# InternRobotics/InternNav

Measured on AMD Instinct MI355X. Metric: policy steps/sec/node, higher is better.
Workload: dtype bf16

## Files before the change

internnav_amd/csrc/gemm_skinny.hip:

```cpp
#include "gemm_skinny_core.h"

namespace {

struct SkBf16 {
    static constexpr bool ROW_SCALE = false;
    using Q = void;
    using S = void;

    template <int MF, int NT16, int NW, int DEPTH>
    static __device__ __forceinline__ void main_fused(const GemmArgs& p, const void*, const void*, int n0, int w, int nmine, int r16, int g,
                                                      f32x4 (&acc)[NT16][MF]) {
        const bf16* __restrict__ A = reinterpret_cast<const bf16*>(p.A);
        const bf16* __restrict__ W = reinterpret_cast<const bf16*>(p.W);
        const bf16x8 zero8 = {0, 0, 0, 0, 0, 0, 0, 0};
        const bf16* wrow[NT16];
        bool wok[NT16];
#pragma unroll
        for (int t = 0; t < NT16; ++t) {
            const int wn = n0 + t * 16 + r16;
            wok[t] = wn < p.N;
            wrow[t] = W + (size_t)(wok[t] ? wn : 0) * p.ldw;
        }
        const bf16* arow[MF];
        bool aok[MF];
#pragma unroll
        for (int i = 0; i < MF; ++i) {
            const int m = i * 16 + r16;
            aok[i] = m < p.M;
            arow[i] = A + (size_t)(aok[i] ? m : 0) * p.lda;
        }
        bf16x8 wf[DEPTH][NT16][4], af[DEPTH][MF][4];
        auto load = [&](int j, int slot) {
            const int k0 = (w + j * NW) * SK_BK + g * 8;
#pragma unroll
            for (int s = 0; s < 4; ++s) {
                const int k = k0 + s * 32;
                const bool kok = j < nmine && k < p.K;
#pragma unroll
                for (int t = 0; t < NT16; ++t) wf[slot][t][s] = (kok && wok[t]) ? *reinterpret_cast<const bf16x8*>(wrow[t] + k) : zero8;
#pragma unroll
                for (int i = 0; i < MF; ++i) af[slot][i][s] = (kok && aok[i]) ? *reinterpret_cast<const bf16x8*>(arow[i] + k) : zero8;
            }
        };
#pragma unroll
        for (int d = 0; d < DEPTH; ++d) load(d, d);
        for (int j0 = 0; j0 < nmine; j0 += DEPTH) {
#pragma unroll
            for (int d = 0; d < DEPTH; ++d) {
#pragma unroll
                for (int t = 0; t < NT16; ++t)
#pragma unroll
                    for (int i = 0; i < MF; ++i)
#pragma unroll
                        for (int s = 0; s < 4; ++s) acc[t][i] = __builtin_amdgcn_mfma_f32_16x16x32_bf16(wf[d][t][s], af[d][i][s], acc[t][i], 0, 0, 0);
                load(j0 + d + DEPTH, d);
            }
        }
    }

    template <int NT16, int NW, int DEPTH, class Norm>
    static __device__ __forceinline__ void main_prenorm(const GemmArgs& p, const void*, const void*, const bf16* img, int lds_ld, int n0, int w,
                                                        int nmine, int r16, int g, f32x4 (&acc)[NT16][1], Norm norm) {
        const bf16* __restrict__ W = reinterpret_cast<const bf16*>(p.W);
        const bf16x8 zero8 = {0, 0, 0, 0, 0, 0, 0, 0};
        const bf16* wrow[NT16];
        bool wok[NT16];
#pragma unroll
        for (int t = 0; t < NT16; ++t) {
            const int wn = n0 + t * 16 + r16;
            wok[t] = wn < p.N;
            wrow[t] = W + (size_t)(wok[t] ? wn : 0) * p.ldw;
        }
        bf16x8 wf[DEPTH][NT16][4];
        auto load_w = [&](int j, int slot) {
            const int k0 = (w + j * NW) * SK_BK + g * 8;
#pragma unroll
            for (int s = 0; s < 4; ++s) {
                const int k = k0 + s * 32;
                const bool kok = j < nmine && k < p.K;
#pragma unroll
                for (int t = 0; t < NT16; ++t) wf[slot][t][s] = (kok && wok[t]) ? *reinterpret_cast<const bf16x8*>(wrow[t] + k) : zero8;
            }
        };
#pragma unroll
        for (int d = 0; d < DEPTH; ++d) load_w(d, d);
        norm();
        const bf16* arow = img + (size_t)(r16 < p.M ? r16 : p.M - 1) * lds_ld + g * 8;
        for (int j0 = 0; j0 < nmine; j0 += DEPTH) {
#pragma unroll
            for (int d = 0; d < DEPTH; ++d) {
                const int kb = (w + (j0 + d) * NW) * SK_BK;
#pragma unroll
                for (int s = 0; s < 4; ++s) {
                    const int k = kb + s * 32;
                    const bf16x8 af = (j0 + d < nmine && k + g * 8 < p.K) ? *reinterpret_cast<const bf16x8*>(arow + k) : zero8;
#pragma unroll
                    for (int t = 0; t < NT16; ++t) acc[t][0] = __builtin_amdgcn_mfma_f32_16x16x32_bf16(wf[d][t][s], af, acc[t][0], 0, 0, 0);
                }
                load_w(j0 + d + DEPTH, d);
            }
        }
    }
};

}

int ina_launch_gemm_skinny_fused(const GemmArgs& p, hipStream_t stream) {
    InaProfScope prof(INA_PROF_GEMM_SKINNY, 2.0 * p.M * p.N * p.K, sk_prof_bytes(p, 2.0 * p.N * p.K), stream);
    return sk_launch_fused<SkBf16>(p, nullptr, nullptr, stream);
}

int ina_launch_gemm_skinny_prenorm(const GemmArgs& p, hipStream_t stream) {
// ... 4 lines not shown
```

internnav_amd/csrc/gemm_skinny_core.h:

```cpp
#pragma once
#include "common.h"
#include "kernels.h"

namespace {

constexpr int SK_BK = 128;

inline int sk_group_waves(int tiles, int ksteps) {
    int nw = tiles >= 4096 ? 1 : tiles >= 2048 ? 2 : tiles >= 1024 ? 4 : 8;
    while (nw > 1 && nw > ksteps) nw >>= 1;
    return nw;
}
inline int sk_group_waves_prenorm(int tiles, int ksteps) {
    const int nw = sk_group_waves(tiles, ksteps);
    return nw < 4 ? 4 : nw;
}

template <int NWAVES>
__device__ __forceinline__ void sk_prenorm_rows(const GemmArgs& p, bf16* img, int lds_ld, int wave, int lane) {
    const int nch = p.K >> 3;
    const float invK = 1.0f / (float)p.K;
    const bool a32 = p.a_dtype == INA_DT_F32;
    auto load8 = [&](int m, int c, float (&v)[8]) {
        if (a32) {
            const float* q = reinterpret_cast<const float*>(p.A) + (size_t)m * p.lda + c * 8;
            const f32x4 a = *reinterpret_cast<const f32x4*>(q), b = *reinterpret_cast<const f32x4*>(q + 4);
#pragma unroll
            for (int j = 0; j < 4; ++j) { v[j] = a[j]; v[4 + j] = b[j]; }
        } else {
            const bf16x8 a = *reinterpret_cast<const bf16x8*>(reinterpret_cast<const bf16*>(p.A) + (size_t)m * p.lda + c * 8);
#pragma unroll
            for (int j = 0; j < 8; ++j) v[j] = (float)a[j];
        }
    };
    for (int m = wave; m < p.M; m += NWAVES) {
        float sq = 0.f;
        for (int c = lane; c < nch; c += 64) {
            float v[8];
            load8(m, c, v);
#pragma unroll
            for (int j = 0; j < 8; ++j) sq = fmaf(v[j], v[j], sq);
        }
        const float rstd = rsqrtf(fmaf(wave_sum(sq), invK, p.norm_eps));
        for (int c = lane; c < nch; c += 64) {
            float v[8];
            load8(m, c, v);
            const f32x4 ga = *reinterpret_cast<const f32x4*>(p.norm_gamma + c * 8), gb = *reinterpret_cast<const f32x4*>(p.norm_gamma + c * 8 + 4);
            bf16x8 o;
#pragma unroll
            for (int j = 0; j < 4; ++j) {
                o[j] = (bf16)(v[j] * rstd * ga[j]);
                o[4 + j] = (bf16)(v[4 + j] * rstd * gb[j]);
            }
            *reinterpret_cast<bf16x8*>(img + (size_t)m * lds_ld + c * 8) = o;
        }
    }
}

template <class I, int MF, int NT16, int NW>
__device__ __forceinline__ void sk_reduce_put(float* red, int grp, int w, int lane, const f32x4 (&acc)[NT16][MF]) {
#pragma unroll
    for (int t = 0; t < NT16; ++t)
#pragma unroll
        for (int i = 0; i < MF; ++i) *reinterpret_cast<f32x4*>(&red[((((I)grp * NW + w) * NT16 + t) * MF + i) * 256 + lane * 4]) = acc[t][i];
}
template <class I, int MF, int NT16, int NW>
__device__ __forceinline__ void sk_reduce_get(const float* red, int grp, int i, int lane, const f32x4 (&acc)[NT16][MF], f32x4 (&sum)[NT16]) {
#pragma unroll
    for (int t = 0; t < NT16; ++t) {
        if constexpr (NW > 1) {
            sum[t] = f32x4{0.f, 0.f, 0.f, 0.f};
#pragma unroll
            for (int ww = 0; ww < NW; ++ww) {
                const f32x4 v = *reinterpret_cast<const f32x4*>(&red[((((I)grp * NW + ww) * NT16 + t) * MF + i) * 256 + lane * 4]);
#pragma unroll
                for (int r = 0; r < 4; ++r) sum[t][r] += v[r];
            }
        } else {
            sum[t] = acc[t][i];
        }
    }
}

template <int NT16>
__device__ __forceinline__ void sk_epilogue(const GemmArgs& p, const f32x4 (&sum)[NT16], int m, int n, int n0, int g) {
    const float rs = p.rowscale ? p.rowscale[m / p.rowscale_div] : 1.0f;
    float v[4];
    int no = n;
    if constexpr (NT16 == 2) {
        no = (n0 >> 1) + g * 4;
#pragma unroll
        for (int r = 0; r < 4; ++r) {
            float gg = sum[0][r], uu = sum[1][r];
            if (p.bias) { gg += p.bias[n + r]; uu += p.bias[n + 16 + r]; }
            v[r] = ina_act(gg, p.act) * uu * rs;
        }
    } else {
#pragma unroll
        for (int r = 0; r < 4; ++r) {
            float x = sum[0][r];
            if (p.bias) x += p.bias[n + r];
            x = ina_act(x, p.act);
            if (p.colscale) x *= p.colscale[n + r];
            v[r] = x * rs;
        }
        if (p.R) {
            const size_t ro = (size_t)m * p.ldr + n;
            if (p.res_dtype == INA_DT_BF16) {
                const bf16x4 rr = *reinterpret_cast<const bf16x4*>(reinterpret_cast<const bf16*>(p.R) + ro);
#pragma unroll
                for (int r = 0; r < 4; ++r) v[r] += (float)rr[r];
            } else {
                const f32x4 rr = *reinterpret_cast<const f32x4*>(reinterpret_cast<const float*>(p.R) + ro);
#pragma unroll
                for (int r = 0; r < 4; ++r) v[r] += rr[r];
            }
        }
    }
    const size_t co = (size_t)m * p.ldc + no;
    if (p.out_dtype == INA_DT_BF16) *reinterpret_cast<bf16x4*>(reinterpret_cast<bf16*>(p.C) + co) = bf16x4{(bf16)v[0], (bf16)v[1], (bf16)v[2], (bf16)v[3]};
    else *reinterpret_cast<f32x4*>(reinterpret_cast<float*>(p.C) + co) = f32x4{v[0], v[1], v[2], v[3]};
}

template <class Fmt, int NT16>
__device__ __forceinline__ void sk_scale_store(const GemmArgs& p, const typename Fmt::S* __restrict__ ws, f32x4 (&sum)[NT16], int m, int n, int n0, int g) {
    if constexpr (Fmt::ROW_SCALE) {
#pragma unroll
        for (int t = 0; t < NT16; ++t)
#pragma unroll
            for (int r = 0; r < 4; ++r) sum[t][r] *= Fmt::row_scale(ws, n + t * 16 + r);
    }
    sk_epilogue<NT16>(p, sum, m, n, n0, g);
}

template <class Fmt, int MF, int NT16, int NW, int NC, int DEPTH>
__global__ __launch_bounds__(NW * NC * 64) void gemm_skinny_fused_kernel(GemmArgs p, const typename Fmt::Q* __restrict__ wq, const typename Fmt::S* __restrict__ ws) {
    __shared__ __attribute__((aligned(16))) float red[(NW > 1 ? NC * NW : 1) * NT16 * MF * 64 * 4];
    const int lane = threadIdx.x & 63, wave = threadIdx.x >> 6;
    const int grp = wave / NW, w = wave % NW;
    const int n0 = (blockIdx.x * NC + grp) * (16 * NT16);
    const int r16 = lane & 15, g = lane >> 4;
    f32x4 acc[NT16][MF];
#pragma unroll
    for (int t = 0; t < NT16; ++t)
#pragma unroll
        for (int i = 0; i < MF; ++i) acc[t][i] = f32x4{0.f, 0.f, 0.f, 0.f};
    const int ksteps = (p.K + SK_BK - 1) / SK_BK;
    const int nmine = w < ksteps ? (ksteps - w + NW - 1) / NW : 0;
    Fmt::template main_fused<MF, NT16, NW, DEPTH>(p, wq, ws, n0, w, nmine, r16, g, acc);
    if constexpr (NW > 1) {
        sk_reduce_put<int, MF, NT16, NW>(red, grp, w, lane, acc);
        __syncthreads();
    }
#pragma unroll
    for (int i = 0; i < MF; ++i) {
        if (NW > 1 && (i % NW) != w) continue;
        const int m = i * 16 + r16, n = n0 + g * 4;
        f32x4 sum[NT16];
        sk_reduce_get<int, MF, NT16, NW>(red, grp, i, lane, acc, sum);
        if (m >= p.M || n >= p.N) continue;
        sk_scale_store<Fmt, NT16>(p, ws, sum, m, n, n0, g);
    }
}

template <class Fmt, int NT16, int NW, int NC, int DEPTH>
__global__ __launch_bounds__(NW * NC * 64) void gemm_skinny_prenorm_kernel(GemmArgs p, const typename Fmt::Q* __restrict__ wq, const typename Fmt::S* __restrict__ ws) {
    extern __shared__ __attribute__((aligned(16))) char sk_smem[];
    constexpr int NWAVES = NW * NC;
    const int lds_ld = p.K + 8;
    bf16* img = reinterpret_cast<bf16*>(sk_smem);
    float* red = reinterpret_cast<float*>(sk_smem + (((size_t)p.M * lds_ld * sizeof(bf16) + 15) & ~size_t(15)));
    const int lane = threadIdx.x & 63, wave = __builtin_amdgcn_readfirstlane(threadIdx.x >> 6);
    const int grp = wave / NW, w = wave % NW;
    const int n0 = (blockIdx.x * NC + grp) * (16 * NT16);
    const int r16 = lane & 15, g = lane >> 4;
    f32x4 acc[NT16][1];
#pragma unroll
    for (int t = 0; t < NT16; ++t) acc[t][0] = f32x4{0.f, 0.f, 0.f, 0.f};
    const int ksteps = (p.K + SK_BK - 1) / SK_BK;
    const int nmine = w < ksteps ? (ksteps - w + NW - 1) / NW : 0;
    Fmt::template main_prenorm<NT16, NW, DEPTH>(p, wq, ws, img, lds_ld, n0, w, nmine, r16, g, acc, [&]() {
        sk_prenorm_rows<NWAVES>(p, img, lds_ld, wave, lane);
        __syncthreads();
    });
    if constexpr (NW > 1) {
        sk_reduce_put<size_t, 1, NT16, NW>(red, grp, w, lane, acc);
        __syncthreads();
        if (w != 0) return;
    }
    const int m = r16, n = n0 + g * 4;
    f32x4 sum[NT16];
    sk_reduce_get<size_t, 1, NT16, NW>(red, grp, 0, lane, acc, sum);
    if (m >= p.M || n >= p.N) return;
    sk_scale_store<Fmt, NT16>(p, ws, sum, m, n, n0, g);
}

template <class Fmt, int MF, int NT16>
void sk_launch_fused_tile(const GemmArgs& p, const typename Fmt::Q* wq, const typename Fmt::S* ws, hipStream_t stream) {
    const int ksteps = (p.K + SK_BK - 1) / SK_BK;
    const int tiles = (p.N + 16 * NT16 - 1) / (16 * NT16);
    const int nw = sk_group_waves(tiles, ksteps);
    constexpr int DEEP = (MF <= 2 && NT16 == 1) ? 4 : 2;
#define INA_SKF(NW_, NC_, D_) \
    hipLaunchKernelGGL((gemm_skinny_fused_kernel<Fmt, MF, NT16, NW_, NC_, D_>), dim3((tiles + NC_ - 1) / NC_), dim3(NW_ * NC_ * 64), 0, stream, p, wq, ws)
    if (nw == 1) INA_SKF(1, 4, 2);
    else if (nw == 2) INA_SKF(2, 2, 2);
    else if (nw == 4) INA_SKF(4, 1, 2);
    else INA_SKF(8, 1, DEEP);
#undef INA_SKF
}

template <class Fmt, int NT16>
int sk_launch_fused_glu(const GemmArgs& p, const typename Fmt::Q* wq, const typename Fmt::S* ws, hipStream_t stream) {
    switch ((p.M + 15) / 16) {
        case 1: sk_launch_fused_tile<Fmt, 1, NT16>(p, wq, ws, stream); break;
        case 2: sk_launch_fused_tile<Fmt, 2, NT16>(p, wq, ws, stream); break;
        case 3: sk_launch_fused_tile<Fmt, 3, NT16>(p, wq, ws, stream); break;
        default: sk_launch_fused_tile<Fmt, 4, NT16>(p, wq, ws, stream); break;
    }
    INA_HIP_CHECK(hipGetLastError());
    return 0;
}
template <class Fmt>
int sk_launch_fused(const GemmArgs& p, const typename Fmt::Q* wq, const typename Fmt::S* ws, hipStream_t stream) {
    return p.glu ? sk_launch_fused_glu<Fmt, 2>(p, wq, ws, stream) : sk_launch_fused_glu<Fmt, 1>(p, wq, ws, stream);
}

template <class Fmt, int NT16, int NW, int NC, int DEPTH>
int sk_launch_prenorm_cfg(const GemmArgs& p, const typename Fmt::Q* wq, const typename Fmt::S* ws, hipStream_t stream, int tiles) {
    const size_t lds = (((size_t)p.M * (p.K + 8) * sizeof(bf16) + 15) & ~size_t(15)) + (NW > 1 ? size_t(NC) * NW * NT16 * 256 * sizeof(float) : 0);
    auto kern = gemm_skinny_prenorm_kernel<Fmt, NT16, NW, NC, DEPTH>;
    static size_t attr = 0;
    if (lds > attr) {
        INA_HIP_CHECK(hipFuncSetAttribute(reinterpret_cast<const void*>(kern), hipFuncAttributeMaxDynamicSharedMemorySize, (int)lds));
        attr = lds;
    }
    hipLaunchKernelGGL(kern, dim3((tiles + NC - 1) / NC), dim3(NW * NC * 64), lds, stream, p, wq, ws);
    INA_HIP_CHECK(hipGetLastError());
    return 0;
}
template <class Fmt>
int sk_launch_prenorm(const GemmArgs& p, const typename Fmt::Q* wq, const typename Fmt::S* ws, hipStream_t stream) {
    const int ksteps = (p.K + SK_BK - 1) / SK_BK;
    if (p.glu) {
        const int tiles = (p.N + 31) / 32;
        if (sk_group_waves_prenorm(tiles, ksteps) == 4) return sk_launch_prenorm_cfg<Fmt, 2, 4, 2, 2>(p, wq, ws, stream, tiles);
        return sk_launch_prenorm_cfg<Fmt, 2, 8, 1, 2>(p, wq, ws, stream, tiles);
    }
    const int tiles = (p.N + 15) / 16;
    if (sk_group_waves_prenorm(tiles, ksteps) == 4) return sk_launch_prenorm_cfg<Fmt, 1, 4, 2, 2>(p, wq, ws, stream, tiles);
    return sk_launch_prenorm_cfg<Fmt, 1, 8, 1, 4>(p, wq, ws, stream, tiles);
}

inline double sk_prof_bytes(const GemmArgs& p, double weight_bytes) {
    const double osz = p.out_dtype == INA_DT_BF16 ? 2.0 : 4.0, asz = (p.norm_gamma && p.a_dtype == INA_DT_F32) ? 4.0 : 2.0;
    return asz * p.M * p.K + weight_bytes + osz * p.M * (p.glu ? p.N / 2 : p.N);
}

template <class LayoutChecks>
int sk_plan_packed(const GemmArgs& p_in, GemmArgs& p, const char* tag, const char* what, LayoutChecks layout) {
    p = p_in;
    if (p.rowscale_div <= 0) p.rowscale_div = 1;
    if (p.batch <= 0) p.batch = 1;
    INA_REQUIRE(p.M > 0 && p.N > 0 && p.K > 0, "%s: empty problem M=%d N=%d K=%d", tag, p.M, p.N, p.K);
    INA_REQUIRE(p.M <= 64, "%s: the %s-weight kernels are weight-streaming kernels for M <= 64 rows (M=%d)", tag, what, p.M);
    INA_REQUIRE(p.K % 128 == 0, "%s: the packed %s layout needs K %% 128 == 0 (K=%d)", tag, what, p.K);
    INA_REQUIRE(p.batch == 1, "%s: no batched form (batch=%d)", tag, p.batch);
    INA_REQUIRE(!p.seg_stats, "%s: seg_stats exist in the row-panel kernels only", tag);
    INA_REQUIRE(!p.Wp, "%s: Wp (fragment-ordered bf16 weights) has no meaning here", tag);
    INA_REQUIRE(p.force_cfg == 0 || p.force_cfg == -1, "%s: no tile configs to force (force_cfg %d)", tag, p.force_cfg);
    if (int rc = layout(p)) return rc;
    INA_REQUIRE(p.lda % 8 == 0, "%s: lda must be a multiple of 8 (lda=%d)", tag, p.lda);
    INA_REQUIRE(p.N % 4 == 0 && p.ldc % 4 == 0, "%s: N/ldc must be multiples of 4 (N=%d ldc=%d)", tag, p.N, p.ldc);
    INA_REQUIRE(((uintptr_t)p.A % 16) == 0 && ((uintptr_t)p.C % 8) == 0, "%s: misaligned pointer", tag);
    INA_REQUIRE(!p.R || p.ldr % 4 == 0, "%s: ldr must be a multiple of 4", tag);
    INA_REQUIRE(!p.glu || (p.N % 32 == 0), "%s: GLU mode needs N %% 32 == 0", tag);
    INA_REQUIRE(p.act >= INA_ACT_NONE && p.act <= INA_ACT_TANH, "%s: act=%d is not an activation code (0 .. %d)", tag, p.act, (int)INA_ACT_TANH);
    INA_REQUIRE(!p.glu || !p.R, "%s: glu cannot be combined with a residual (R)", tag);
    INA_REQUIRE(!p.glu || !p.colscale, "%s: glu cannot be combined with colscale", tag);
    if (p.norm_gamma) {
        INA_REQUIRE(p.M <= 16 && p.K <= 4096 && p.N >= 256,
                    "%s: the fused input RMSNorm is built for the decode passes (M <= 16 rows, K <= 4096): M=%d K=%d N=%d", tag, p.M, p.K, p.N);
        INA_REQUIRE(p.a_dtype == INA_DT_BF16 || p.a_dtype == INA_DT_F32, "%s: a_dtype must be bf16 or f32 with norm_gamma", tag);
        INA_REQUIRE(((uintptr_t)p.norm_gamma % 16) == 0 && (p.lda % (p.a_dtype == INA_DT_F32 ? 4 : 8)) == 0, "%s(prenorm): misaligned gamma / lda", tag);
    }
    return 0;
}

}
```

internnav_amd/csrc/gemm_skinny_mx4.hip:

```cpp
#include "gemm_skinny_core.h"

namespace {

typedef unsigned int u32x4 __attribute__((ext_vector_type(4)));

__device__ __forceinline__ bf16x8 mx4_frag(unsigned int q, unsigned int scale_byte) {
    const float sc = __uint_as_float(scale_byte << 23);
    const bf16x2 a = __builtin_amdgcn_cvt_scalef32_pk_bf16_fp4(q, sc, 0), b = __builtin_amdgcn_cvt_scalef32_pk_bf16_fp4(q, sc, 1);
    const bf16x2 c = __builtin_amdgcn_cvt_scalef32_pk_bf16_fp4(q, sc, 2), d = __builtin_amdgcn_cvt_scalef32_pk_bf16_fp4(q, sc, 3);
    return bf16x8{a[0], a[1], b[0], b[1], c[0], c[1], d[0], d[1]};
}
__device__ __forceinline__ unsigned int mx4_scale_byte(unsigned int four, int s) { return (four >> (8 * s)) & 0xffu; }

constexpr int MX_BKB = 64;

struct SkMx4 {
    static constexpr bool ROW_SCALE = false;
    using Q = uint8_t;
    using S = uint8_t;

    template <int MF, int NT16, int NW, int DEPTH>
    static __device__ __forceinline__ void main_fused(const GemmArgs& p, const uint8_t* __restrict__ W4, const uint8_t* __restrict__ wscale, int n0, int w, int nmine,
                                                      int r16, int g, f32x4 (&acc)[NT16][MF]) {
        const bf16* __restrict__ A = reinterpret_cast<const bf16*>(p.A);
        const bf16x8 zero8 = {0, 0, 0, 0, 0, 0, 0, 0};
        const u32x4 zero4 = {0u, 0u, 0u, 0u};
        const int spitch = p.K >> 5;
        const uint8_t* wrow[NT16];
        const uint8_t* srow[NT16];
        bool wok[NT16];
#pragma unroll
        for (int t = 0; t < NT16; ++t) {
            const int wn = n0 + t * 16 + r16;
            wok[t] = wn < p.N;
            wrow[t] = W4 + (size_t)(wok[t] ? wn : 0) * p.ldw + g * 16;
            srow[t] = wscale + (size_t)(wok[t] ? wn : 0) * spitch;
        }
        const bf16* arow[MF];
        bool aok[MF];
#pragma unroll
        for (int i = 0; i < MF; ++i) {
            const int m = i * 16 + r16;
            aok[i] = m < p.M;
            arow[i] = A + (size_t)(aok[i] ? m : 0) * p.lda;
        }
        u32x4 wf[DEPTH][NT16];
        unsigned int ws[DEPTH][NT16];
        bf16x8 af[DEPTH][MF][4];
        auto load = [&](int j, int slot) {
            const bool kok = j < nmine;
            const int ks = w + j * NW;
#pragma unroll
            for (int t = 0; t < NT16; ++t) {
                wf[slot][t] = (kok && wok[t]) ? *reinterpret_cast<const u32x4*>(wrow[t] + (size_t)ks * MX_BKB) : zero4;
                ws[slot][t] = (kok && wok[t]) ? *reinterpret_cast<const unsigned int*>(srow[t] + ks * 4) : 0u;
            }
            const int kb = ks * SK_BK;
#pragma unroll
            for (int s = 0; s < 4; ++s)
#pragma unroll
                for (int i = 0; i < MF; ++i) af[slot][i][s] = (kok && aok[i]) ? *reinterpret_cast<const bf16x8*>(arow[i] + kb + s * 32 + g * 8) : zero8;
        };
#pragma unroll
        for (int d = 0; d < DEPTH; ++d) load(d, d);
        for (int j0 = 0; j0 < nmine; j0 += DEPTH) {
#pragma unroll
            for (int d = 0; d < DEPTH; ++d) {
                if (j0 + d >= nmine) break;
#pragma unroll
                for (int t = 0; t < NT16; ++t) {
                    bf16x8 wb[4];
#pragma unroll
                    for (int s = 0; s < 4; ++s) wb[s] = mx4_frag(wf[d][t][s], mx4_scale_byte(ws[d][t], s));
#pragma unroll
                    for (int i = 0; i < MF; ++i)
#pragma unroll
                        for (int s = 0; s < 4; ++s) acc[t][i] = __builtin_amdgcn_mfma_f32_16x16x32_bf16(wb[s], af[d][i][s], acc[t][i], 0, 0, 0);
                }
                load(j0 + d + DEPTH, d);
            }
        }
    }

    template <int NT16, int NW, int DEPTH, class Norm>
    static __device__ __forceinline__ void main_prenorm(const GemmArgs& p, const uint8_t* __restrict__ W4, const uint8_t* __restrict__ wscale, const bf16* img,
                                                        int lds_ld, int n0, int w, int nmine, int r16, int g, f32x4 (&acc)[NT16][1], Norm norm) {
        const u32x4 zero4 = {0u, 0u, 0u, 0u};
        const int spitch = p.K >> 5;
        const uint8_t* wrow[NT16];
        const uint8_t* srow[NT16];
        bool wok[NT16];
#pragma unroll
        for (int t = 0; t < NT16; ++t) {
            const int wn = n0 + t * 16 + r16;
            wok[t] = wn < p.N;
            wrow[t] = W4 + (size_t)(wok[t] ? wn : 0) * p.ldw + g * 16;
            srow[t] = wscale + (size_t)(wok[t] ? wn : 0) * spitch;
        }
        u32x4 wf[DEPTH][NT16];
        unsigned int ws[DEPTH][NT16];
        auto load_w = [&](int j, int slot) {
            const bool kok = j < nmine;
            const int ks = w + j * NW;
#pragma unroll
            for (int t = 0; t < NT16; ++t) {
                wf[slot][t] = (kok && wok[t]) ? *reinterpret_cast<const u32x4*>(wrow[t] + (size_t)ks * MX_BKB) : zero4;
                ws[slot][t] = (kok && wok[t]) ? *reinterpret_cast<const unsigned int*>(srow[t] + ks * 4) : 0u;
            }
        };
#pragma unroll
        for (int d = 0; d < DEPTH; ++d) load_w(d, d);
        norm();
        const bf16* arow = img + (size_t)(r16 < p.M ? r16 : p.M - 1) * lds_ld + g * 8;
        for (int j0 = 0; j0 < nmine; j0 += DEPTH) {
#pragma unroll
            for (int d = 0; d < DEPTH; ++d) {
                if (j0 + d >= nmine) break;
                const int kb = (w + (j0 + d) * NW) * SK_BK;
#pragma unroll
                for (int s = 0; s < 4; ++s) {
                    const bf16x8 af = *reinterpret_cast<const bf16x8*>(arow + kb + s * 32);
#pragma unroll
                    for (int t = 0; t < NT16; ++t)
                        acc[t][0] = __builtin_amdgcn_mfma_f32_16x16x32_bf16(mx4_frag(wf[d][t][s], mx4_scale_byte(ws[d][t], s)), af, acc[t][0], 0, 0, 0);
                }
                load_w(j0 + d + DEPTH, d);
            }
// ... 27 lines not shown
```

internnav_amd/csrc/gemm_skinny_w8.hip:

```cpp
#include "gemm_skinny_core.h"

namespace {

typedef unsigned int u32x4 __attribute__((ext_vector_type(4)));

__device__ __forceinline__ bf16x8 w8_frag(unsigned int lo, unsigned int hi) {
    const bf16x2 a = __builtin_amdgcn_cvt_scalef32_pk_bf16_fp8(lo, 1.0f, false), b = __builtin_amdgcn_cvt_scalef32_pk_bf16_fp8(lo, 1.0f, true);
    const bf16x2 c = __builtin_amdgcn_cvt_scalef32_pk_bf16_fp8(hi, 1.0f, false), d = __builtin_amdgcn_cvt_scalef32_pk_bf16_fp8(hi, 1.0f, true);
    return bf16x8{a[0], a[1], b[0], b[1], c[0], c[1], d[0], d[1]};
}

struct SkFp8 {
    static constexpr bool ROW_SCALE = true;
    using Q = uint8_t;
    using S = int8_t;
    static __device__ __forceinline__ float row_scale(const int8_t* __restrict__ wexp, int n) { return __int_as_float((127 + wexp[n]) << 23); }

    template <int MF, int NT16, int NW, int DEPTH>
    static __device__ __forceinline__ void main_fused(const GemmArgs& p, const uint8_t* __restrict__ W8, const int8_t*, int n0, int w, int nmine, int r16, int g,
                                                      f32x4 (&acc)[NT16][MF]) {
        const bf16* __restrict__ A = reinterpret_cast<const bf16*>(p.A);
        const bf16x8 zero8 = {0, 0, 0, 0, 0, 0, 0, 0};
        const u32x4 zero4 = {0u, 0u, 0u, 0u};
        const uint8_t* wrow[NT16];
        bool wok[NT16];
#pragma unroll
        for (int t = 0; t < NT16; ++t) {
            const int wn = n0 + t * 16 + r16;
            wok[t] = wn < p.N;
            wrow[t] = W8 + (size_t)(wok[t] ? wn : 0) * p.ldw + g * 32;
        }
        const bf16* arow[MF];
        bool aok[MF];
#pragma unroll
        for (int i = 0; i < MF; ++i) {
            const int m = i * 16 + r16;
            aok[i] = m < p.M;
            arow[i] = A + (size_t)(aok[i] ? m : 0) * p.lda;
        }
        u32x4 wf[DEPTH][NT16][2];
        bf16x8 af[DEPTH][MF][4];
        auto load = [&](int j, int slot) {
            const bool kok = j < nmine;
            const int kb = (w + j * NW) * SK_BK;
#pragma unroll
            for (int t = 0; t < NT16; ++t)
#pragma unroll
                for (int h = 0; h < 2; ++h) wf[slot][t][h] = (kok && wok[t]) ? *reinterpret_cast<const u32x4*>(wrow[t] + kb + h * 16) : zero4;
#pragma unroll
            for (int s = 0; s < 4; ++s)
#pragma unroll
                for (int i = 0; i < MF; ++i) af[slot][i][s] = (kok && aok[i]) ? *reinterpret_cast<const bf16x8*>(arow[i] + kb + s * 32 + g * 8) : zero8;
        };
#pragma unroll
        for (int d = 0; d < DEPTH; ++d) load(d, d);
        for (int j0 = 0; j0 < nmine; j0 += DEPTH) {
#pragma unroll
            for (int d = 0; d < DEPTH; ++d) {
#pragma unroll
                for (int t = 0; t < NT16; ++t) {
                    bf16x8 wb[4];
#pragma unroll
                    for (int s = 0; s < 4; ++s) wb[s] = w8_frag(wf[d][t][s >> 1][(s & 1) * 2], wf[d][t][s >> 1][(s & 1) * 2 + 1]);
#pragma unroll
                    for (int i = 0; i < MF; ++i)
#pragma unroll
                        for (int s = 0; s < 4; ++s) acc[t][i] = __builtin_amdgcn_mfma_f32_16x16x32_bf16(wb[s], af[d][i][s], acc[t][i], 0, 0, 0);
                }
                load(j0 + d + DEPTH, d);
            }
        }
    }

    template <int NT16, int NW, int DEPTH, class Norm>
    static __device__ __forceinline__ void main_prenorm(const GemmArgs& p, const uint8_t* __restrict__ W8, const int8_t*, const bf16* img, int lds_ld, int n0,
                                                        int w, int nmine, int r16, int g, f32x4 (&acc)[NT16][1], Norm norm) {
        const bf16x8 zero8 = {0, 0, 0, 0, 0, 0, 0, 0};
        const u32x4 zero4 = {0u, 0u, 0u, 0u};
        const uint8_t* wrow[NT16];
        bool wok[NT16];
#pragma unroll
        for (int t = 0; t < NT16; ++t) {
            const int wn = n0 + t * 16 + r16;
            wok[t] = wn < p.N;
            wrow[t] = W8 + (size_t)(wok[t] ? wn : 0) * p.ldw + g * 32;
        }
        u32x4 wf[DEPTH][NT16][2];
        auto load_w = [&](int j, int slot) {
            const bool kok = j < nmine;
            const int kb = (w + j * NW) * SK_BK;
#pragma unroll
            for (int t = 0; t < NT16; ++t)
#pragma unroll
                for (int h = 0; h < 2; ++h) wf[slot][t][h] = (kok && wok[t]) ? *reinterpret_cast<const u32x4*>(wrow[t] + kb + h * 16) : zero4;
        };
#pragma unroll
        for (int d = 0; d < DEPTH; ++d) load_w(d, d);
        norm();
        const bf16* arow = img + (size_t)(r16 < p.M ? r16 : p.M - 1) * lds_ld + g * 8;
        for (int j0 = 0; j0 < nmine; j0 += DEPTH) {
#pragma unroll
            for (int d = 0; d < DEPTH; ++d) {
                const int kb = (w + (j0 + d) * NW) * SK_BK;
#pragma unroll
                for (int s = 0; s < 4; ++s) {
                    const bf16x8 af = (j0 + d < nmine) ? *reinterpret_cast<const bf16x8*>(arow + kb + s * 32) : zero8;
#pragma unroll
                    for (int t = 0; t < NT16; ++t)
                        acc[t][0] = __builtin_amdgcn_mfma_f32_16x16x32_bf16(w8_frag(wf[d][t][s >> 1][(s & 1) * 2], wf[d][t][s >> 1][(s & 1) * 2 + 1]), af, acc[t][0], 0, 0, 0);
                }
                load_w(j0 + d + DEPTH, d);
            }
        }
    }
};

}

int ina_plan_gemm_w8(const GemmArgs& p_in, const void* W8, const int8_t* wexp, GemmArgs& p) {
    INA_REQUIRE(W8 != nullptr && wexp != nullptr, "gemm_w8: null weight / exponent pointer");
    return sk_plan_packed(p_in, p, "gemm_w8", "fp8", [&](const GemmArgs& q) {
// ... 16 lines not shown
```

internnav_amd/qwen_vl.py:

```python
from __future__ import annotations

import weakref
from types import SimpleNamespace
from typing import Dict, List, Optional, Sequence, Tuple

import numpy as np
import torch

from . import ops
from .runtime import CapacityError


def vision_window_permutation(grids: Sequence[Tuple[int, int, int]], merge: int = 2, window: int = 112, patch: int = 14):
    win = window // merge // patch
    idx_all, cu, base = [], [0], 0
    for t, h, w in grids:
        gh, gw = h // merge, w // merge
        idx = np.arange(t * gh * gw).reshape(t, gh, gw)
        ph, pw = win - gh % win, win - gw % win
        nh, nw = (gh + ph) // win, (gw + pw) // win
        pad = np.pad(idx, ((0, 0), (0, ph), (0, pw)), constant_values=-100)
        pad = pad.reshape(t, nh, win, nw, win).transpose(0, 1, 3, 2, 4).reshape(t, nh * nw, win * win)
        lens = (pad != -100).sum(-1).reshape(-1)
        flat = pad.reshape(-1)
# ... 400 lines not shown

    def refresh_w8_weights(self):
        if self.mx4_decode:
            raise ValueError("refresh_w8_weights on an mx4_decode engine: drop_mx4_weights() first (the weights would be rounded twice)")
        for L in self.layers:
            for k in self.W8_LAYER_WEIGHTS:
                w8, e, wd = ops.w8_quantize(L[k])
                L[k].copy_(wd)
                L[k + "8"] = (w8, e)
        w8, e, wd = ops.w8_quantize(self.lm_head)
        self.lm_head.copy_(wd)
        self.lm_head8 = (w8, e)
        self.w8_decode = True
        if self.frag_weights:
            self.refresh_frag_weights()

    def drop_w8_weights(self):
        self.w8_decode = False
        self.lm_head8 = None
        for L in self.layers:
            for k in self.W8_LAYER_WEIGHTS:
                L.pop(k + "8", None)

    def refresh_mx4_weights(self):
        if self.w8_decode:
            raise ValueError("refresh_mx4_weights on a w8_decode engine: drop_w8_weights() first (the weights would be rounded twice)")
        for L in self.layers:
            for k in self.W8_LAYER_WEIGHTS:
                w4, sc, wd = ops.mx4_quantize(L[k])
                L[k].copy_(wd)
                L[k + "4"] = (w4, sc)
        w8, e, wd = ops.w8_quantize(self.lm_head)
        self.lm_head.copy_(wd)
        self.lm_head8 = (w8, e)
        self.mx4_decode = True
        if self.frag_weights:
            self.refresh_frag_weights()

    def drop_mx4_weights(self):
        self.mx4_decode = False
        self.lm_head8 = None
        for L in self.layers:
            for k in self.W8_LAYER_WEIGHTS:
                L.pop(k + "4", None)

    def _linear(self, x, L: dict, k: str, quant, **kw):
        if quant:
            kw.pop("w_frag", None)
            if quant == "4":
                return ops.linear_mx4(x, *L[k + "4"], **kw)
            return ops.linear_w8(x, *L[k + "8"], **kw)
        return ops.linear(x, L[k], **kw)

    def _phase(self, B: int, S: int, pos3: np.ndarray, cache_pos0, k_len: Optional[np.ndarray] = None, b0: int = 0) -> dict:
        dev = self.device
        pos0 = np.broadcast_to(np.asarray(cache_pos0, dtype=np.int64).reshape(-1, 1), (B, 1))
        rows = ((b0 + np.arange(B))[:, None] * self.S_max + pos0 + np.arange(S)[None]).reshape(-1).astype(np.int32)
        if int(pos0.max()) + S > self.S_max:
            raise CapacityError(f"KV cache capacity exceeded: {int(pos0.max()) + S} tokens > max_seq_len={self.S_max}")
        ph = dict(B=B, S=S, pos=torch.from_numpy(np.ascontiguousarray(np.broadcast_to(pos3, (3, B, S)).reshape(3, B * S)).astype(np.int32)).to(dev),
                  rows=torch.from_numpy(rows).to(dev), Lk=int(pos0.max()) + S, k_len=None, b0=b0, r0=b0 * S)
        if k_len is not None:
            ph["k_len"] = torch.from_numpy(np.asarray(k_len, dtype=np.int32)).to(dev)
        ph["new_are_last"] = bool(np.all((np.asarray(k_len).reshape(-1) if k_len is not None else ph["Lk"]) == pos0[:, 0] + S))
        ph["w0"] = pos0[:, 0].copy()
        return ph

    def _layers(self, ph: dict):
        H, nh, nkv, hd, Smax = self.H, self.nh, self.nkv, self.hd, self.S_max
        B, S = ph["B"], ph["S"]
        rows, r0, b0 = B * S, ph.get("r0", 0), ph.get("b0", 0)
        if self._kv_views and "w0" in ph:
            self._kv_evict({b0 + i: int(w) for i, w in enumerate(ph["w0"])})
        x, h, att, qkv, ff, x_in, cos, sin = (t[r0:r0 + rows] for t in (self.x, self.h, self.att, self.qkv, self.ff, self.x_in, self.cos, self.sin))
        ops.mrope_table(ph["pos"], self.inv_freq, self.axis_of, cos, sin)
        q4 = qkv[:, : nh * hd].view(B, S, nh, hd)
        single = rows <= 16 and self.tap is None
        fused_norm = single and self.fuse_decode_norm
        pfx = ph.get("prefix")
        if pfx is not None:
            k4 = qkv[:, nh * hd:(nh + nkv) * hd].view(B, S, nkv, hd)
            v4 = qkv[:, (nh + nkv) * hd:].view(B, S, nkv, hd)
        shr = ph.get("shared")
        fuse_rope = pfx is None and shr is None and single and self.fuse_decode_rope and ph.get("new_are_last", False) and ops.attention_rope_ok(S, ph["Lk"], nh, nkv, hd)
        if fuse_rope:
            kn4 = qkv[:, nh * hd:(nh + nkv) * hd].view(B, S, nkv, hd)
            vn4 = qkv[:, (nh + nkv) * hd:].view(B, S, nkv, hd)
        quant = ("8" if self.w8_decode else "4" if self.mx4_decode else None) if rows <= SKINNY_GEMM_MAX_ROWS else None
        for li, L in enumerate(self.layers):
            src = x_in if li == 0 else x
            wf = (lambda k, L=L: L.get(k)) if (self.frag_weights and rows > SKINNY_GEMM_MAX_ROWS) else (lambda k: None)
            if fused_norm:
                self._linear(src, L, "qkv_w", quant, bias=L["qkv_b"], out=qkv, prenorm=(L["n1"], 1e-6))
            else:
                ops.norm(src, L["n1"], None, eps=1e-6, rms=True, out=h)
                self._linear(h, L, "qkv_w", quant, bias=L["qkv_b"], out=qkv, w_frag=wf("qkv_wf"))
            if pfx is not None:
                ops.rope(qkv, cos, sin, heads=nh + nkv, D=hd, col0=0, rows=rows)
                kvc = L["kv"].view(self.B_max, Smax, 2, nkv, hd)
                tl = pfx.get("tail")
                if tl is None:
                    ops.attention_prefix(q4, k4, v4, kvc[:, :, 0], kvc[:, :, 1], pfx["slot"], pfx["pfx_len"], pfx["suf_len"],
                                         out=att.view(B, S, nh, hd), max_pfx=pfx["max_pfx"])
                else:
                    t5 = tl["tails"][li][: tl["rows"] * tl["T"]].view(tl["rows"], tl["T"], 2, nkv, hd)
                    ops.attention_prefix_tail(q4, k4, v4, kvc[:, :, 0], kvc[:, :, 1], pfx["slot"], pfx["pfx_len"], pfx["suf_len"], t5[:, :, 0],
                                              t5[:, :, 1], tl["tail_row"], tl["tail_len"], out=att.view(B, S, nh, hd), max_pfx=pfx["max_pfx"],
                                              max_tail=tl["max_tail"])
            elif shr is not None:
                tail = shr["tails"][li]
                ops.rope(qkv, cos, sin, heads=nh + nkv, D=hd, col0=0, rows=rows, kv_out=tail, kv_dst=shr["kv_dst"], kv_head0=nh, v_heads=nkv)
                kvc = L["kv"].view(self.B_max, Smax, 2, nkv, hd)
                t5 = tail[: rows * shr["T"]].view(rows, shr["T"], 2, nkv, hd)
                ops.attention_shared(qkv[:, : nh * hd].view(rows, nh, hd), t5[:, :, 0], t5[:, :, 1], kvc[:, :, 0], kvc[:, :, 1], shr["tile_rows"],
                                     shr["tile_slot"], shr["tile_pfx"], shr["tail_len"], out=att.view(rows, nh, hd), max_pfx=shr["max_pfx"])
            else:
                if not fuse_rope:
                    ops.rope(qkv, cos, sin, heads=nh + nkv, D=hd, col0=0, rows=rows, kv_out=L["kv"], kv_dst=ph["rows"], kv_head0=nh, v_heads=nkv)
                kv4 = L["kv"].view(self.B_max, Smax, 2, nkv, hd)[b0:b0 + B, : ph["Lk"]]
                ops.attention(q4, kv4[:, :, 0], kv4[:, :, 1], causal=True, out=att.view(B, S, nh, hd), k_len=ph["k_len"],
                              rope=(cos, sin, kn4, vn4) if fuse_rope else None)
            self._linear(att, L, "o_w", quant, residual=src, out=x)
            if fused_norm:
                self._linear(x, L, "gu_w", quant, act="silu", glu=True, out=ff, prenorm=(L["n2"], 1e-6))
            else:
                ops.norm(x, L["n2"], None, eps=1e-6, rms=True, out=h)
                self._linear(h, L, "gu_w", quant, act="silu", glu=True, out=ff, w_frag=wf("gu_wf"))
            self._linear(ff, L, "down_w", quant, residual=x, out=x, w_frag=wf("down_wf"))
            if self.tap is not None:
                self.tap("llm", li, x)

    def _suffix_phase(self, slot, next_pos, pfx_len, suf_len, m: int, tail_row=None, tail_len=None) -> dict:
        dev = self.device
        slot, pfx_len, suf_len = (np.asarray(v, dtype=np.int64).reshape(-1) for v in (slot, pfx_len, suf_len))
        P = slot.size
        assert P >= 1 and pfx_len.size == P and suf_len.size == P and np.asarray(next_pos).size == P
        if not 1 <= m <= ops.ATTN_PREFIX_MAX_ROWS:
            raise ValueError(f"a suffix pass runs 1 .. {ops.ATTN_PREFIX_MAX_ROWS} tokens per pair, got {m}")
        if P * m > self.x.shape[0]:
            raise CapacityError(f"suffix pass of {P} x {m} tokens exceeds the engine's {self.x.shape[0]} buffer rows")
        assert int(slot.min()) >= 0 and int(slot.max()) < self.B_max and int(pfx_len.min()) >= 0 and int(pfx_len.max()) <= self.S_max
        assert int(suf_len.min()) >= 0 and int(suf_len.max()) <= m
        pos = (np.asarray(next_pos, dtype=np.int64).reshape(-1, 1) + np.arange(m)[None]).reshape(1, P * m)
        i32 = lambda v: torch.from_numpy(np.ascontiguousarray(v).astype(np.int32)).to(dev)
        prefix = dict(slot=i32(slot), pfx_len=i32(pfx_len), suf_len=i32(suf_len), max_pfx=int(pfx_len.max()))
        if tail_row is not None:
            bufs = self._shared
            tail_row, tail_len = (np.asarray(v, dtype=np.int64).reshape(-1) for v in (tail_row, tail_len))
            assert bufs is not None and tail_row.size == P and tail_len.size == P
            assert int(tail_row.min()) >= 0 and int(tail_row.max()) < bufs.rows and int(tail_len.min()) >= 0 and int(tail_len.max()) <= bufs.T
            prefix["tail"] = dict(tails=bufs.tails, rows=bufs.rows, T=bufs.T, tail_row=i32(tail_row), tail_len=i32(tail_len), max_tail=int(tail_len.max()))
        return dict(B=P, S=m, pos=i32(np.broadcast_to(pos, (3, P * m))), b0=0, r0=0, prefix=prefix)

    def suffix_pass(self, state: dict, prompt_of, tokens, suf_len) -> torch.Tensor:
        tokens = np.asarray(tokens, dtype=np.int64)
        P, m = tokens.shape
        prompt_of = np.asarray(prompt_of, dtype=np.int64).reshape(-1)
        assert prompt_of.size == P and int(prompt_of.min()) >= 0 and int(prompt_of.max()) < state["B"]
        lens = state.get("lens")
        pl = np.full(state["B"], state["S"], dtype=np.int64) if lens is None else np.asarray(lens, dtype=np.int64)
        ph = self._suffix_phase(prompt_of, np.asarray(state["next_pos"])[prompt_of], pl[prompt_of], suf_len, m)
        ops.gather_rows(self.embed, self.x_in, src=torch.from_numpy(tokens.reshape(-1).astype(np.int32)).to(self.device), rows=P * m)
        self._layers(ph)
        return self.x[: P * m]

    def _last_logits(self, B: int, S: int, row_in_seq, rows_idx: Optional[torch.Tensor] = None, penalty: Optional[float] = None, col: int = 0,
                     sampling: Optional[dict] = None, src: Optional[torch.Tensor] = None, bufs=None):
# ... 584 lines not shown
```

Baseline: 302.7.

## Stage skinny-GEMM activations through per-wave LDS with coalesced row loads

For skinny GEMM configs with at least two M-fragments and 8x1 or 4x2 wave layouts, activation tiles are now loaded with a coalesced row-major pattern, written to a per-wave LDS image, and read back as MFMA fragments. The next tile's load is software-pipelined behind the current compute. The reduction buffer overlays the dynamic staging memory, which costs an extra block barrier. Other changes: deeper weight prefetch (DEPTH 4) for all NT16==1 tiles, and rope fusion allowed beyond single-row decode.

```diff
diff --git a/internnav_amd/csrc/gemm_skinny.hip b/internnav_amd/csrc/gemm_skinny.hip
--- a/internnav_amd/csrc/gemm_skinny.hip
+++ b/internnav_amd/csrc/gemm_skinny.hip
@@ -9,7 +9,7 @@
 
     template <int MF, int NT16, int NW, int DEPTH>
     static __device__ __forceinline__ void main_fused(const GemmArgs& p, const void*, const void*, int n0, int w, int nmine, int r16, int g,
-                                                      f32x4 (&acc)[NT16][MF]) {
+                                                      bf16* stage, f32x4 (&acc)[NT16][MF]) {
         const bf16* __restrict__ A = reinterpret_cast<const bf16*>(p.A);
         const bf16* __restrict__ W = reinterpret_cast<const bf16*>(p.W);
         const bf16x8 zero8 = {0, 0, 0, 0, 0, 0, 0, 0};
@@ -28,6 +28,42 @@
             const int m = i * 16 + r16;
             aok[i] = m < p.M;
             arow[i] = A + (size_t)(aok[i] ? m : 0) * p.lda;
+        }
+        if constexpr (sk_act_staged(MF, NT16, NW)) {
+            const int lane = g * 16 + r16;
+            bf16x8 wf[DEPTH][NT16][4], ar[MF * 4];
+            auto load_w = [&](int j, int slot) {
+                const int k0 = (w + j * NW) * SK_BK + g * 8;
+#pragma unroll
+                for (int s = 0; s < 4; ++s) {
+                    const int k = k0 + s * 32;
+                    const bool kok = j < nmine && k < p.K;
+#pragma unroll
+                    for (int t = 0; t < NT16; ++t) wf[slot][t][s] = (kok && wok[t]) ? *reinterpret_cast<const bf16x8*>(wrow[t] + k) : zero8;
+                }
+            };
+            load_w(0, 0);
+            sk_stage_load<MF>(A, p, w * SK_BK, 0 < nmine, lane, ar);
+#pragma unroll
+            for (int d = 1; d < DEPTH; ++d) load_w(d, d);
+            for (int j0 = 0; j0 < nmine; j0 += DEPTH) {
+#pragma unroll
+                for (int d = 0; d < DEPTH; ++d) {
+                    sk_stage_put<MF>(stage, lane, ar);
+                    sk_stage_load<MF>(A, p, (w + (j0 + d + 1) * NW) * SK_BK, j0 + d + 1 < nmine, lane, ar);
+#pragma unroll
+                    for (int i = 0; i < MF; ++i)
+#pragma unroll
+                        for (int s = 0; s < 4; ++s) {
+                            const bf16x8 af = sk_stage_get(stage, i, s, r16, g);
+#pragma unroll
+                            for (int t = 0; t < NT16; ++t) acc[t][i] = __builtin_amdgcn_mfma_f32_16x16x32_bf16(wf[d][t][s], af, acc[t][i], 0, 0, 0);
+                        }
+                    sk_stage_done();
+                    load_w(j0 + d + DEPTH, d);
+                }
+            }
+            return;
         }
         bf16x8 wf[DEPTH][NT16][4], af[DEPTH][MF][4];
         auto load = [&](int j, int slot) {
diff --git a/internnav_amd/csrc/gemm_skinny_core.h b/internnav_amd/csrc/gemm_skinny_core.h
--- a/internnav_amd/csrc/gemm_skinny_core.h
+++ b/internnav_amd/csrc/gemm_skinny_core.h
@@ -14,6 +14,34 @@
 inline int sk_group_waves_prenorm(int tiles, int ksteps) {
     const int nw = sk_group_waves(tiles, ksteps);
     return nw < 4 ? 4 : nw;
+}
+
+constexpr int SK_ST_LD = SK_BK + 8;
+constexpr bool sk_act_staged(int MF, int NT16, int NW) { return MF >= 2 && ((NT16 == 1 && NW == 8) || (NT16 == 2 && NW == 4)); }
+constexpr size_t sk_stage_bytes(int MF, int NT16, int NW, int NC) { return sk_act_staged(MF, NT16, NW) ? (size_t)NW * NC * MF * 16 * SK_ST_LD * sizeof(bf16) : 0; }
+
+template <int MF>
+__device__ __forceinline__ void sk_stage_load(const bf16* __restrict__ A, const GemmArgs& p, int kb, bool kok, int lane, bf16x8 (&ar)[MF * 4]) {
+    const bf16x8 zero8 = {0, 0, 0, 0, 0, 0, 0, 0};
+    const int c = lane & 15, rr = lane >> 4;
+    const bool cok = kok && kb + c * 8 < p.K;
+#pragma unroll
+    for (int q = 0; q < MF * 4; ++q) {
+        const int m = q * 4 + rr;
+        ar[q] = (cok && m < p.M) ? *reinterpret_cast<const bf16x8*>(A + (size_t)m * p.lda + kb + c * 8) : zero8;
+    }
+}
+template <int MF>
+__device__ __forceinline__ void sk_stage_put(bf16* img, int lane, const bf16x8 (&ar)[MF * 4]) {
+    const int c = lane & 15, rr = lane >> 4;
+#pragma unroll
+    for (int q = 0; q < MF * 4; ++q) *reinterpret_cast<bf16x8*>(img + (q * 4 + rr) * SK_ST_LD + c * 8) = ar[q];
+    __builtin_amdgcn_fence(__ATOMIC_ACQ_REL, "wavefront");
+    __builtin_amdgcn_wave_barrier();
+}
+__device__ __forceinline__ void sk_stage_done() { __builtin_amdgcn_fence(__ATOMIC_ACQ_REL, "wavefront"); }
+__device__ __forceinline__ bf16x8 sk_stage_get(const bf16* img, int i, int s, int r16, int g) {
+    return *reinterpret_cast<const bf16x8*>(img + (i * 16 + r16) * SK_ST_LD + s * 32 + g * 8);
 }
 
 template <int NWAVES>
@@ -135,9 +163,13 @@
 
 template <class Fmt, int MF, int NT16, int NW, int NC, int DEPTH>
 __global__ __launch_bounds__(NW * NC * 64) void gemm_skinny_fused_kernel(GemmArgs p, const typename Fmt::Q* __restrict__ wq, const typename Fmt::S* __restrict__ ws) {
-    __shared__ __attribute__((aligned(16))) float red[(NW > 1 ? NC * NW : 1) * NT16 * MF * 64 * 4];
+    constexpr bool STAGED = sk_act_staged(MF, NT16, NW);
+    extern __shared__ __attribute__((aligned(16))) char sk_smem[];
+    __shared__ __attribute__((aligned(16))) float red_own[STAGED ? 4 : (NW > 1 ? NC * NW : 1) * NT16 * MF * 64 * 4];
+    float* red = STAGED ? reinterpret_cast<float*>(sk_smem) : red_own;
     const int lane = threadIdx.x & 63, wave = threadIdx.x >> 6;
     const int grp = wave / NW, w = wave % NW;
+    bf16* stage = STAGED ? reinterpret_cast<bf16*>(sk_smem) + (size_t)wave * (MF * 16 * SK_ST_LD) : nullptr;
     const int n0 = (blockIdx.x * NC + grp) * (16 * NT16);
     const int r16 = lane & 15, g = lane >> 4;
     f32x4 acc[NT16][MF];
@@ -147,8 +179,10 @@
         for (int i = 0; i < MF; ++i) acc[t][i] = f32x4{0.f, 0.f, 0.f, 0.f};
     const int ksteps = (p.K + SK_BK - 1) / SK_BK;
     const int nmine = w < ksteps ? (ksteps - w + NW - 1) / NW : 0;
-    Fmt::template main_fused<MF, NT16, NW, DEPTH>(p, wq, ws, n0, w, nmine, r16, g, acc);
+    Fmt::template main_fused<MF, NT16, NW, DEPTH>(p, wq, ws, n0, w, nmine, r16, g, stage, acc);
     if constexpr (NW > 1) {
+        static_assert(!STAGED || sizeof(float) * NT16 * 64 * 4 <= sizeof(bf16) * 16 * SK_ST_LD, "the reduction buffer fits the images it lies over");
+        if constexpr (STAGED) __syncthreads();
         sk_reduce_put<int, MF, NT16, NW>(red, grp, w, lane, acc);
         __syncthreads();
     }
@@ -195,14 +229,28 @@
     sk_scale_store<Fmt, NT16>(p, ws, sum, m, n, n0, g);
 }
 
+template <class Fmt, int MF, int NT16, int NW, int NC, int DEPTH>
+int sk_launch_fused_cfg(const GemmArgs& p, const typename Fmt::Q* wq, const typename Fmt::S* ws, hipStream_t stream, int tiles) {
+    constexpr size_t lds = sk_stage_bytes(MF, NT16, NW, NC);
+    auto kern = gemm_skinny_fused_kernel<Fmt, MF, NT16, NW, NC, DEPTH>;
+    if constexpr (lds > 48 * 1024) {
+        static bool allowed = false;
+        if (!allowed) {
+            INA_HIP_CHECK(hipFuncSetAttribute(reinterpret_cast<const void*>(kern), hipFuncAttributeMaxDynamicSharedMemorySize, (int)lds));
+            allowed = true;
+        }
+    }
+    hipLaunchKernelGGL(kern, dim3((tiles + NC - 1) / NC), dim3(NW * NC * 64), lds, stream, p, wq, ws);
+    return 0;
+}
+
 template <class Fmt, int MF, int NT16>
-void sk_launch_fused_tile(const GemmArgs& p, const typename Fmt::Q* wq, const typename Fmt::S* ws, hipStream_t stream) {
+int sk_launch_fused_tile(const GemmArgs& p, const typename Fmt::Q* wq, const typename Fmt::S* ws, hipStream_t stream) {
     const int ksteps = (p.K + SK_BK - 1) / SK_BK;
     const int tiles = (p.N + 16 * NT16 - 1) / (16 * NT16);
     const int nw = sk_group_waves(tiles, ksteps);
-    constexpr int DEEP = (MF <= 2 && NT16 == 1) ? 4 : 2;
-#define INA_SKF(NW_, NC_, D_) \
-    hipLaunchKernelGGL((gemm_skinny_fused_kernel<Fmt, MF, NT16, NW_, NC_, D_>), dim3((tiles + NC_ - 1) / NC_), dim3(NW_ * NC_ * 64), 0, stream, p, wq, ws)
+    constexpr int DEEP = NT16 == 1 ? 4 : 2;
+#define INA_SKF(NW_, NC_, D_) return sk_launch_fused_cfg<Fmt, MF, NT16, NW_, NC_, D_>(p, wq, ws, stream, tiles)
     if (nw == 1) INA_SKF(1, 4, 2);
     else if (nw == 2) INA_SKF(2, 2, 2);
     else if (nw == 4) INA_SKF(4, 1, 2);
@@ -212,12 +260,14 @@
 
 template <class Fmt, int NT16>
 int sk_launch_fused_glu(const GemmArgs& p, const typename Fmt::Q* wq, const typename Fmt::S* ws, hipStream_t stream) {
+    int rc = 0;
     switch ((p.M + 15) / 16) {
-        case 1: sk_launch_fused_tile<Fmt, 1, NT16>(p, wq, ws, stream); break;
-        case 2: sk_launch_fused_tile<Fmt, 2, NT16>(p, wq, ws, stream); break;
-        case 3: sk_launch_fused_tile<Fmt, 3, NT16>(p, wq, ws, stream); break;
-        default: sk_launch_fused_tile<Fmt, 4, NT16>(p, wq, ws, stream); break;
-    }
+        case 1: rc = sk_launch_fused_tile<Fmt, 1, NT16>(p, wq, ws, stream); break;
+        case 2: rc = sk_launch_fused_tile<Fmt, 2, NT16>(p, wq, ws, stream); break;
+        case 3: rc = sk_launch_fused_tile<Fmt, 3, NT16>(p, wq, ws, stream); break;
+        default: rc = sk_launch_fused_tile<Fmt, 4, NT16>(p, wq, ws, stream); break;
+    }
+    if (rc) return rc;
     INA_HIP_CHECK(hipGetLastError());
     return 0;
 }
diff --git a/internnav_amd/csrc/gemm_skinny_mx4.hip b/internnav_amd/csrc/gemm_skinny_mx4.hip
--- a/internnav_amd/csrc/gemm_skinny_mx4.hip
+++ b/internnav_amd/csrc/gemm_skinny_mx4.hip
@@ -21,7 +21,7 @@
 
     template <int MF, int NT16, int NW, int DEPTH>
     static __device__ __forceinline__ void main_fused(const GemmArgs& p, const uint8_t* __restrict__ W4, const uint8_t* __restrict__ wscale, int n0, int w, int nmine,
-                                                      int r16, int g, f32x4 (&acc)[NT16][MF]) {
+                                                      int r16, int g, bf16* stage, f32x4 (&acc)[NT16][MF]) {
         const bf16* __restrict__ A = reinterpret_cast<const bf16*>(p.A);
         const bf16x8 zero8 = {0, 0, 0, 0, 0, 0, 0, 0};
         const u32x4 zero4 = {0u, 0u, 0u, 0u};
@@ -43,6 +43,49 @@
             const int m = i * 16 + r16;
             aok[i] = m < p.M;
             arow[i] = A + (size_t)(aok[i] ? m : 0) * p.lda;
+        }
+        if constexpr (sk_act_staged(MF, NT16, NW)) {
+            const int lane = g * 16 + r16;
+            u32x4 wf[DEPTH][NT16];
+            unsigned int ws[DEPTH][NT16];
+            bf16x8 ar[MF * 4];
+            auto load_w = [&](int j, int slot) {
+                const bool kok = j < nmine;
+                const int ks = w + j * NW;
+#pragma unroll
+                for (int t = 0; t < NT16; ++t) {
+                    wf[slot][t] = (kok && wok[t]) ? *reinterpret_cast<const u32x4*>(wrow[t] + (size_t)ks * MX_BKB) : zero4;
+                    ws[slot][t] = (kok && wok[t]) ? *reinterpret_cast<const unsigned int*>(srow[t] + ks * 4) : 0u;
+                }
+            };
+            load_w(0, 0);
+            sk_stage_load<MF>(A, p, w * SK_BK, 0 < nmine, lane, ar);
+#pragma unroll
+            for (int d = 1; d < DEPTH; ++d) load_w(d, d);
+            for (int j0 = 0; j0 < nmine; j0 += DEPTH) {
+#pragma unroll
+                for (int d = 0; d < DEPTH; ++d) {
+                    if (j0 + d >= nmine) break;
+                    sk_stage_put<MF>(stage, lane, ar);
+                    sk_stage_load<MF>(A, p, (w + (j0 + d + 1) * NW) * SK_BK, j0 + d + 1 < nmine, lane, ar);
+                    bf16x8 wb[NT16][4];
+#pragma unroll
+                    for (int t = 0; t < NT16; ++t)
+#pragma unroll
+                        for (int s = 0; s < 4; ++s) wb[t][s] = mx4_frag(wf[d][t][s], mx4_scale_byte(ws[d][t], s));
+#pragma unroll
+                    for (int i = 0; i < MF; ++i)
+#pragma unroll
+                        for (int s = 0; s < 4; ++s) {
+                            const bf16x8 af = sk_stage_get(stage, i, s, r16, g);
+#pragma unroll
+                            for (int t = 0; t < NT16; ++t) acc[t][i] = __builtin_amdgcn_mfma_f32_16x16x32_bf16(wb[t][s], af, acc[t][i], 0, 0, 0);
+                        }
+                    sk_stage_done();
+                    load_w(j0 + d + DEPTH, d);
+                }
+            }
+            return;
         }
         u32x4 wf[DEPTH][NT16];
         unsigned int ws[DEPTH][NT16];
diff --git a/internnav_amd/csrc/gemm_skinny_w8.hip b/internnav_amd/csrc/gemm_skinny_w8.hip
--- a/internnav_amd/csrc/gemm_skinny_w8.hip
+++ b/internnav_amd/csrc/gemm_skinny_w8.hip
@@ -18,7 +18,7 @@
 
     template <int MF, int NT16, int NW, int DEPTH>
     static __device__ __forceinline__ void main_fused(const GemmArgs& p, const uint8_t* __restrict__ W8, const int8_t*, int n0, int w, int nmine, int r16, int g,
-                                                      f32x4 (&acc)[NT16][MF]) {
+                                                      bf16* stage, f32x4 (&acc)[NT16][MF]) {
         const bf16* __restrict__ A = reinterpret_cast<const bf16*>(p.A);
         const bf16x8 zero8 = {0, 0, 0, 0, 0, 0, 0, 0};
         const u32x4 zero4 = {0u, 0u, 0u, 0u};
@@ -37,6 +37,46 @@
             const int m = i * 16 + r16;
             aok[i] = m < p.M;
             arow[i] = A + (size_t)(aok[i] ? m : 0) * p.lda;
+        }
+        if constexpr (sk_act_staged(MF, NT16, NW)) {
+            const int lane = g * 16 + r16;
+            u32x4 wf[DEPTH][NT16][2];
+            bf16x8 ar[MF * 4];
+            auto load_w = [&](int j, int slot) {
+                const bool kok = j < nmine;
+                const int kb = (w + j * NW) * SK_BK;
+#pragma unroll
+                for (int t = 0; t < NT16; ++t)
+#pragma unroll
+                    for (int h = 0; h < 2; ++h) wf[slot][t][h] = (kok && wok[t]) ? *reinterpret_cast<const u32x4*>(wrow[t] + kb + h * 16) : zero4;
+            };
+            load_w(0, 0);
+            sk_stage_load<MF>(A, p, w * SK_BK, 0 < nmine, lane, ar);
+#pragma unroll
+            for (int d = 1; d < DEPTH; ++d) load_w(d, d);
+            for (int j0 = 0; j0 < nmine; j0 += DEPTH) {
+#pragma unroll
+                for (int d = 0; d < DEPTH; ++d) {
+                    sk_stage_put<MF>(stage, lane, ar);
+                    sk_stage_load<MF>(A, p, (w + (j0 + d + 1) * NW) * SK_BK, j0 + d + 1 < nmine, lane, ar);
+                    bf16x8 wb[NT16][4];
+#pragma unroll
+                    for (int t = 0; t < NT16; ++t)
+#pragma unroll
+                        for (int s = 0; s < 4; ++s) wb[t][s] = w8_frag(wf[d][t][s >> 1][(s & 1) * 2], wf[d][t][s >> 1][(s & 1) * 2 + 1]);
+#pragma unroll
+                    for (int i = 0; i < MF; ++i)
+#pragma unroll
+                        for (int s = 0; s < 4; ++s) {
+                            const bf16x8 af = sk_stage_get(stage, i, s, r16, g);
+#pragma unroll
+                            for (int t = 0; t < NT16; ++t) acc[t][i] = __builtin_amdgcn_mfma_f32_16x16x32_bf16(wb[t][s], af, acc[t][i], 0, 0, 0);
+                        }
+                    sk_stage_done();
+                    load_w(j0 + d + DEPTH, d);
+                }
+            }
+            return;
         }
         u32x4 wf[DEPTH][NT16][2];
         bf16x8 af[DEPTH][MF][4];
diff --git a/internnav_amd/qwen_vl.py b/internnav_amd/qwen_vl.py
--- a/internnav_amd/qwen_vl.py
+++ b/internnav_amd/qwen_vl.py
@@ -506,7 +506,8 @@
             k4 = qkv[:, nh * hd:(nh + nkv) * hd].view(B, S, nkv, hd)
             v4 = qkv[:, (nh + nkv) * hd:].view(B, S, nkv, hd)
         shr = ph.get("shared")
-        fuse_rope = pfx is None and shr is None and single and self.fuse_decode_rope and ph.get("new_are_last", False) and ops.attention_rope_ok(S, ph["Lk"], nh, nkv, hd)
+        fuse_rope = (pfx is None and shr is None and self.tap is None and self.fuse_decode_rope and ph.get("new_are_last", False)
+                     and ops.attention_rope_ok(S, ph["Lk"], nh, nkv, hd))
         if fuse_rope:
             kn4 = qkv[:, nh * hd:(nh + nkv) * hd].view(B, S, nkv, hd)
             vn4 = qkv[:, (nh + nkv) * hd:].view(B, S, nkv, hd)
```

After: 304.1, median of 6. Within noise of the previous version (+0.5%).
